# ricardo0115/p-div-gnn

Measured on AMD Instinct MI355X. Metric: mesh-nodes/sec (fwd+bwd) on periodic FEM graphs, higher is better.
Workload: dtype f32

## Files before the change

include/pdivgnn.h:

```cpp
#ifndef PDIVGNN_H
#define PDIVGNN_H

#include <stdint.h>

#ifdef __cplusplus
extern "C" {
#endif

#define PDG_LATENT 128
#define PDG_OK 0
#define PDG_ERR_ARG 1
#define PDG_ERR_HIP 2

typedef struct pdg_ln_stat {
  float mean;
  float den;
  float rstd;
  float std_;
  double mean_d, std_d, count;
} pdg_ln_stat;

typedef struct pdg_ln_bwd {
  float c1, c2;
  double S1, S2;
// ... 22 lines not shown
int pdg_ln_partials_sum(const double* partials, int nparts, double* out2, void* stream);

int pdg_node_pq(int n_nodes, const float* a2_prev, const pdg_ln_stat* st, const float* ln_g,
                const float* ln_b, const float* x_res, float* x_out, const float* W1,
                float* P, float* Q, void* stream);
int pdg_node_pq_rw(int n_nodes, const float* a2_prev, const pdg_ln_stat* st, const float* ln_g,
                   const float* ln_b, const float* x_res, float* x_out, const float* W1, float* P,
                   float* Q, void* stream);
int pdg_node_pq_rw_fin(int n_nodes, const float* a2_prev, const double* partials, int nparts, double count,
                       pdg_ln_stat* st_out, const float* ln_g, const float* ln_b, const float* x_res,
                       float* x_out, const float* W1, float* P, float* Q, void* stream);

int pdg_edge_fwd(int n_edges, const float* a2_prev, const pdg_ln_stat* st, const float* ln_g,
                 const float* ln_b, const float* e_res, float* e_out, const int* src, const int* dst,
                 const float* P, const float* Q, const float* W1, const float* b1,
                 const float* W2, const float* b2, float* a1m, float* a2m, float* a1e, float* a2e,
                 double* part_m, double* part_e, int with_edge_update, int* nparts, void* stream);

int pdg_segment_sum(int n_nodes, const int* rowptr, const float* rows, const pdg_ln_stat* st,
                    const float* ln_g, const float* ln_b, float* out, float* xhat_sum, void* stream);
int pdg_segment_sum_fin(int n_nodes, const int* rowptr, const float* rows, const double* part_a,
                        const double* part_b, int nparts, double count, pdg_ln_stat* st_a, pdg_ln_stat* st_b,
                        const float* ln_g, const float* ln_b, float* out, float* xhat_sum, void* stream);

int pdg_node_mlp1(int n_nodes, const float* aggr, const float* x, const float* Wn1,
                  const float* bn1, float* a1n, void* stream);

int pdg_mlp2_fwd(int rows, const float* a1, const float* W2, const float* b2, float* a2,
                 double* partials, int* nparts, void* stream);

int pdg_node_net(int n_nodes, const float* aggr, const float* x, const float* Wn1, const float* bn1,
                 const float* Wn2, const float* bn2, float* a1n, float* a2n, double* partials,
                 int* nparts, void* stream);
int pdg_decoder_fwd(int n_nodes, const float* a2_prev, const pdg_ln_stat* st, const float* ln_g,
                    const float* ln_b, const float* x_res, float* x_out, const float* Wd1,
                    const float* bd1, float* a1d, const float* Wd2, const float* bd2,
                    const float* stats8, int scale_output, float* y, void* stream);
int pdg_decoder_fwd_fin(int n_nodes, const float* a2_prev, const double* partials, int nparts, double count,
                        pdg_ln_stat* st_out, const float* ln_g, const float* ln_b, const float* x_res,
                        float* x_out, const float* Wd1, const float* bd1, float* a1d, const float* Wd2,
                        const float* bd2, const float* stats8, int scale_output, float* y, void* stream);
int pdg_decoder_fwd_coop(int n_nodes, const float* a2_prev, const pdg_ln_stat* st, const double* partials,
                         int nparts, double count, pdg_ln_stat* st_out, const float* ln_g, const float* ln_b,
                         const float* x_res, float* x_out, const float* Wd1, const float* bd1, float* a1d,
                         const float* Wd2, const float* bd2, const float* stats8, int scale_output, float* y,
                         int nblocks, void* stream);

int pdg_any_nonzero(const float* x, int64_t n, int* flag, void* stream);

int pdg_zero_unless(const int* flag, float* y, int64_t n, void* stream);


int pdg_decoder_bwd(int n_nodes, const float* gy, const float* a1d, const float* Wd2,
                    const float* Wd1T, float* gz1d, float* gx, void* stream);

int pdg_ln_colsum(int rows, const float* gy_rows, const int* gidx, const float* a2,
                  const pdg_ln_stat* st, double* partials, int* nparts, const float* ln_g,
                  double* pairs, int accumulate, void* stream);

int pdg_ln_colsum_nodes(int n_nodes, const float* gaggr, const int* rowptr, const float* xhat_sum,
                        double* partials, int* nparts, const float* ln_g, double* pairs, int accumulate,
                        void* stream);

int pdg_ln_colsum_finalize(const double* partials, int nparts, const float* ln_g,
                           const pdg_ln_stat* st, float* grad_g, float* grad_b, pdg_ln_bwd* out,
                           void* stream);
// ... 182 lines not shown
```

p-div-gnn_amd/csrc/pdg_common.hpp:

```cpp
#pragma once
#include <hip/hip_runtime.h>
#include <stdint.h>

#include "../../include/pdivgnn.h"
#include "pdg_runtime.hpp"

namespace pdg {

constexpr int L = 128;
constexpr int TILE = 16;
constexpr int FRAG = 32;
constexpr int WPAD = 136;
constexpr int WBLK = 128 * WPAD;
#ifndef PDG_EDGE_WAVES
#define PDG_EDGE_WAVES 12
#endif
constexpr int EDGE_WAVES = PDG_EDGE_WAVES;
constexpr float LN_EPS = 1e-5f;

typedef float f32x4 __attribute__((ext_vector_type(4)));
typedef unsigned u32x4 __attribute__((ext_vector_type(4)));

typedef pdg_ln_stat LNStat;
typedef pdg_ln_bwd LNBwd;
// ... 43 lines not shown
#endif
constexpr int PQ_LD = PDG_PQ_BLOCKED ? 2 * 128 : 128;
__device__ __forceinline__ int pq_col(int c) { return PDG_PQ_BLOCKED ? c + (c & ~15) : c; }

__device__ __forceinline__ __amdgpu_buffer_rsrc_t rows_rsrc(float* base, int r0, int r1) {
  return __builtin_amdgcn_make_buffer_rsrc(base ? base + (size_t)r0 * L : nullptr, (short)0,
                                           base ? (r1 - r0) * L * 4 : 0, 0x00020000);
}
__device__ __forceinline__ void rows_store4(__amdgpu_buffer_rsrc_t rs, int r, int c, const f32x4& v) {
  __builtin_amdgcn_raw_buffer_store_b128(__builtin_bit_cast(u32x4, v), rs, (r * L + c) * 4, 0, 0);
}
__device__ __forceinline__ void rows_store4_nt(__amdgpu_buffer_rsrc_t rs, int r, int c, const f32x4& v) {
  __builtin_amdgcn_raw_buffer_store_b128(__builtin_bit_cast(u32x4, v), rs, (r * L + c) * 4, 0, 2);
}

__device__ __forceinline__ void stnt4(float* __restrict__ p, const f32x4& x) { st4(p, 0, x); }
__device__ __forceinline__ float div_den(float x, float den, float rstd) {
  const float q = x * rstd;
  const float r = fmaf(-q, den, x);
  return fmaf(r, rstd, q);
}

template <bool RES>
__device__ __forceinline__ f32x4 ln_res4(const f32x4& x, const f32x4& r, const LNStat& st, const f32x4& g,
                                         const f32x4& b) {
  f32x4 y;
#pragma unroll
  for (int j = 0; j < 4; ++j) {
    float v = div_den(x[j] - st.mean, st.den, st.rstd) * g[j] + b[j];
    if (RES) v += r[j];
    y[j] = v;
  }
  return y;
}

__device__ __forceinline__ void load_wblock(float* __restrict__ lds, const float* __restrict__ W,
                                            int ld, int col0) {
  for (int idx = threadIdx.x; idx < 128 * 32; idx += blockDim.x) {
    const int o = idx >> 5, c4 = idx & 31;
    const f32x4 val = *reinterpret_cast<const f32x4*>(W + (size_t)o * ld + col0 + 4 * c4);
    *reinterpret_cast<f32x4*>(lds + o * WPAD + 4 * c4) = val;
  }
}

struct Acc {
  f32x4 b[8];
};
#define ACC(acc, s) (acc).b[(s) >> 2][(s) & 3]
#define PDG_FOR_FRAG(s) _Pragma("unroll") for (int s = 0; s < FRAG; ++s)
#define PDG_FENCE() __builtin_amdgcn_sched_barrier(0)

__device__ __forceinline__ void zero_acc(Acc& acc) {
#pragma unroll
  for (int ob = 0; ob < 8; ++ob) acc.b[ob] = f32x4{0.f, 0.f, 0.f, 0.f};
}

struct FeatVec {
  float lo, hi;
};
__device__ __forceinline__ FeatVec load_featvec(const float* __restrict__ p) {
  const int l = lane_id();
  return FeatVec{p[l], p[64 + l]};
}
__device__ __forceinline__ f32x4 featvec_chunk(const FeatVec& fv, int T) {
  const int addr = opaque(4 * (16 * (T & 3) + 4 * (lane_id() >> 4)));
  const int src = __float_as_int(T < 4 ? fv.lo : fv.hi);
// ... 295 lines not shown
```

p-div-gnn_amd/csrc/pdg_fwd.hip:

```cpp
#include <stdarg.h>
#include <stdio.h>

#include "pdg_common.hpp"
#include "pdg_runtime.hpp"

using namespace pdg;

namespace pdg {

static thread_local char g_err[512];

void set_error(const char* fmt, ...) {
  va_list ap;
  va_start(ap, fmt);
  vsnprintf(g_err, sizeof(g_err), fmt, ap);
  va_end(ap);
}

int device_cus() {
  static int cached[64] = {0};
  int dev = 0;
  (void)hipGetDevice(&dev);
  if (dev < 0 || dev >= 64) dev = 0;
  if (!cached[dev]) {
// ... 464 lines not shown
  __shared__ double red[8];
  if (part_a) {
    if (blockIdx.x == 0 && part_b) {
      ln_stat_from_partials(part_b, nparts, count, st_b, red);
      __syncthreads();
    }
    ln_stat_from_partials(part_a, nparts, count, &st_sh, red);
    __syncthreads();
    if (blockIdx.x == 0 && threadIdx.x == 0) *st_a = st_sh;
    stp = &st_sh;
  }
  const bool ln = stp != nullptr;
  if (ln) {
    mean = stp->mean;
    den = stp->den;
    rstd = stp->rstd;
    g = reinterpret_cast<const f32x4*>(lg)[j];
    b = reinterpret_cast<const f32x4*>(lb)[j];
  }
  for (int v = blockIdx.x * nhw + hw; v < N; v += gridDim.x * nhw) {
    const int k0 = rowptr[v], k1 = rowptr[v + 1];
    f32x4 acc = {0.f, 0.f, 0.f, 0.f}, xs = {0.f, 0.f, 0.f, 0.f};
    for (int k = k0; k < k1; k += SEG_U) {
      f32x4 x[SEG_U];
#pragma unroll
      for (int u = 0; u < SEG_U; ++u) {
        const int kk = k + u < k1 ? k + u : k1 - 1;
        x[u] = reinterpret_cast<const f32x4*>(rows + (size_t)kk * L)[j];
      }
#pragma unroll
      for (int u = 0; u < SEG_U; ++u) {
        if (k + u >= k1) break;
        if (ln) {
#pragma unroll
          for (int c = 0; c < 4; ++c) {
            const float h = div_den(x[u][c] - mean, den, rstd);
            xs[c] += h;
            x[u][c] = h * g[c] + b[c];
          }
        }
        acc += x[u];
      }
    }
    stg4(out + (size_t)v * L + 4 * j, acc);
    if (xsum) stg4(xsum + (size_t)v * L + 4 * j, xs);
  }
}

extern "C" int pdg_segment_sum(int n_nodes, const int* rowptr, const float* rows, const pdg_ln_stat* st,
                               const float* ln_g, const float* ln_b, float* out, float* xhat_sum, void* stream) {
  PDG_CHECK_ARG(!xhat_sum || (st && PDG_ALIGNED(xhat_sum)), "pdg_segment_sum: xhat_sum needs st, 16-B alignment");
  PDG_CHECK_ARG(n_nodes > 0, "pdg_segment_sum: n_nodes must be > 0");
  PDG_CHECK_ARG(PDG_ALIGNED(rows) && PDG_ALIGNED(out), "pdg_segment_sum: misaligned pointer");
  long want = (n_nodes + 7) / 8;
  long cap = (long)device_cus() * 8;
  const int grid = (int)(want < cap ? want : cap);
  hipLaunchKernelGGL(segment_sum_kernel, dim3(grid), dim3(256), 0, (hipStream_t)stream, n_nodes, rowptr, rows,
                     st, ln_g, ln_b, out, xhat_sum, nullptr, nullptr, 0, 0.0, nullptr, nullptr);
  PDG_CHECK_LAUNCH("pdg_segment_sum");
  return PDG_OK;
}

extern "C" int pdg_segment_sum_fin(int n_nodes, const int* rowptr, const float* rows, const double* part_a,
                                   const double* part_b, int nparts, double count, pdg_ln_stat* st_a,
                                   pdg_ln_stat* st_b, const float* ln_g, const float* ln_b, float* out,
                                   float* xhat_sum, void* stream) {
  PDG_CHECK_ARG(n_nodes > 0, "pdg_segment_sum_fin: n_nodes must be > 0");
  PDG_CHECK_ARG(part_a && st_a && ln_g && ln_b && nparts > 0 && nparts <= MAX_BLOCKS && count > 0 &&
                    (!part_b || st_b),
                "pdg_segment_sum_fin: bad statistics arguments");
  PDG_CHECK_ARG(PDG_ALIGNED(rows) && PDG_ALIGNED(out) && (!xhat_sum || PDG_ALIGNED(xhat_sum)),
                "pdg_segment_sum_fin: misaligned pointer");
// ... 231 lines not shown
```

p-div-gnn_amd/csrc/pdg_node.hip:

```cpp
#include "pdg_common.hpp"
#include "pdg_runtime.hpp"
#include "pdg_x6.hpp"

using namespace pdg;

namespace {

constexpr int NU_COMPUTE = 8;
constexpr int NU_LOADERS = 4;
constexpr int NU_THREADS = 64 * (NU_COMPUTE + NU_LOADERS);
constexpr int XS = 2 * L + 8;
constexpr int AS = L + 8;
constexpr int XBUF = TILE * XS;

struct TileRegs {
  f32x4 v[4];
};

__device__ __forceinline__ void fetch_tile(TileRegs& tr, int t, int N, int lt, const float* __restrict__ aggr,
                                           const float* __restrict__ x) {
  const int j = lt & 31, lr = lt >> 5;
#pragma unroll
  for (int u = 0; u < 4; ++u) {
    const int r = lr + 8 * (u >> 1), node = t * TILE + r;
// ... 105 lines not shown
    }
    stage((i + 2) % 3);
  }
  __shared__ double red[2 * NU_COMPUTE];
  block_sum2(s1, s2, red);
  if (threadIdx.x == 0) {
    part[2 * blockIdx.x] = s1;
    part[2 * blockIdx.x + 1] = s2;
  }
}



extern "C" int pdg_node_net(int n_nodes, const float* aggr, const float* x, const float* Wn1, const float* bn1,
                            const float* Wn2, const float* bn2, float* a1n, float* a2n, double* partials,
                            int* nparts, void* stream) {
  PDG_CHECK_ARG(n_nodes > 0, "pdg_node_net: n_nodes must be > 0");
  PDG_CHECK_ARG(n_nodes < (1 << 22), "pdg_node_net: at most 4,194,303 nodes per call");
  PDG_CHECK_ARG(aggr && x && a2n, "pdg_node_net: aggr, x and a2n are required");
  PDG_CHECK_ARG(PDG_ALIGNED(aggr) && PDG_ALIGNED(x) && PDG_ALIGNED(Wn1) && PDG_ALIGNED(Wn2) && PDG_ALIGNED(a2n) &&
                    PDG_ALIGNED(a1n) && PDG_ALIGNED(bn1) && PDG_ALIGNED(bn2),
                "pdg_node_net: misaligned pointer");
  const int tiles = tiles_of(n_nodes);
  const int cap = device_cus() < MAX_BLOCKS ? device_cus() : MAX_BLOCKS;
  const int grid = tiles < cap ? tiles : cap;
  hipLaunchKernelGGL(node_net_x6_kernel, dim3(grid), dim3(64 * NU_COMPUTE), 0, (hipStream_t)stream, n_nodes, aggr, x,
                     Wn1, bn1, Wn2, bn2, a1n, a2n, partials);
  PDG_CHECK_LAUNCH("pdg_node_net");
  if (nparts) *nparts = grid;
  return PDG_OK;
}

namespace {

constexpr int GS = L + 8;

struct Gz2Regs {
  f32x4 gv[2], av[2];
};

__device__ __forceinline__ void fetch_gz2(Gz2Regs& rg, int t, int N, int lt, const float* __restrict__ gy,
                                          const float* __restrict__ a2) {
#pragma unroll
  for (int u = 0; u < 2; ++u) {
    const int c = lt + 256 * u, rr = c >> 5, j = c & 31, node = t * TILE + rr;
    const bool ok = node < N;
    rg.gv[u] = ok ? reinterpret_cast<const f32x4*>(gy + (size_t)node * L)[j] : f32x4{0.f, 0.f, 0.f, 0.f};
    rg.av[u] = ok ? reinterpret_cast<const f32x4*>(a2 + (size_t)node * L)[j] : f32x4{0.f, 0.f, 0.f, 0.f};
  }
}

__device__ __forceinline__ void store_gz2(float* __restrict__ buf, float* __restrict__ gybuf, int t, int N, int lt,
                                          const Gz2Regs& rg, const LNStat& st, const pdg_ln_bwd& lb,
                                          const float* __restrict__ g, float* __restrict__ gz2_out) {
#pragma unroll
  for (int u = 0; u < 2; ++u) {
    const int c = lt + 256 * u, rr = c >> 5, j = c & 31, node = t * TILE + rr;
    const f32x4 gg = reinterpret_cast<const f32x4*>(g)[j];
    f32x4 z;
#pragma unroll
    for (int e = 0; e < 4; ++e) {
      const float xhat = div_den(rg.av[u][e] - st.mean, st.den, st.rstd);
      const float ga = st.rstd * (gg[e] * rg.gv[u][e] - lb.c1) - xhat * lb.c2;
      z[e] = rg.av[u][e] > 0.f ? ga : 0.f;
    }
    *reinterpret_cast<f32x4*>(buf + rr * GS + 4 * j) = z;
// ... 370 lines not shown
```

p-div-gnn_amd/pdg/engine.py:

```python
from __future__ import annotations

import ctypes
import os
from dataclasses import dataclass, field

import torch

from . import hiptimer
from .lib import LN_STAT_BYTES, lib, stream_handle
from .lib import ptr as _p
from .plan import GraphPlan

L = 128
VP, IA = ctypes.c_void_p, ctypes.c_int


def _arr(ctype, values):
    values = list(values)
    return (ctype * len(values))(*values)


PARAM_SHAPES = [
    ("node_encoder.0.weight", (L, 6)), ("node_encoder.0.bias", (L,)),
    ("node_encoder.2.weight", (L, L)), ("node_encoder.2.bias", (L,)),
    ("node_encoder.4.weight", (L,)), ("node_encoder.4.bias", (L,)),
    ("edge_encoder.0.weight", (L, 1)), ("edge_encoder.0.bias", (L,)),
    ("edge_encoder.2.weight", (L, L)), ("edge_encoder.2.bias", (L,)),
    ("edge_encoder.4.weight", (L,)), ("edge_encoder.4.bias", (L,)),
    ("processor.edge_net.0.weight", (L, 3 * L)), ("processor.edge_net.0.bias", (L,)),
    ("processor.edge_net.2.weight", (L, L)), ("processor.edge_net.2.bias", (L,)),
    ("processor.edge_net.4.weight", (L,)), ("processor.edge_net.4.bias", (L,)),
    ("processor.node_net.0.weight", (L, 2 * L)), ("processor.node_net.0.bias", (L,)),
    ("processor.node_net.2.weight", (L, L)), ("processor.node_net.2.bias", (L,)),
    ("processor.node_net.4.weight", (L,)), ("processor.node_net.4.bias", (L,)),
    ("node_decoder.0.weight", (L, L)), ("node_decoder.0.bias", (L,)),
    ("node_decoder.2.weight", (3, L)), ("node_decoder.2.bias", (3,)),
]
PARAM_NAMES = [n for n, _ in PARAM_SHAPES]


VARIANTS = {
    "fused_edge_wgrad": ("PDG_FUSED_EDGE_WGRAD", True),
    "gz1e_from_gc": ("PDG_GZ1E_FROM_GC", True),
    "coop_fwd": ("PDG_EDGE_FWD_COOP", True),
    "pair_blocks_per_cu": ("PDG_PAIR_BLOCKS_PER_CU", 1),
    "enc_blocks_per_cu": ("PDG_ENC_BLOCKS_PER_CU", 2),
}


INFER_PIPE_MIN_EDGES = 32768


def _parse_variant(name: str, raw: str):
    env, default = VARIANTS[name]
    if isinstance(default, bool):
        if raw not in ("0", "1"):
            raise ValueError(f"{env}={raw!r}: expected 0 or 1")
        return raw == "1"
    try:
        v = int(raw)
    except ValueError:
        raise ValueError(f"{env}={raw!r}: expected an integer") from None
    if v < 1 or v > 4:
        raise ValueError(f"{env}={raw!r}: expected 1..4")
    return v


def kernel_variants(overrides: dict | None = None) -> dict:
    out = {k: d for k, (_, d) in VARIANTS.items()}
    ab = os.environ.get("PDG_AB") == "1"
    for name, (env, default) in VARIANTS.items():
        raw = os.environ.get(env)
        if raw is None:
            continue
        val = _parse_variant(name, raw)
        if val != default and not ab:
            raise RuntimeError(f"{env}={raw} selects a non-default kernel variant of the HIP path; these are "
# ... 90 lines not shown
    n_node: int = 0
    sync_slot: int = 0

    def PN(self, t):
        return self.pairs[t]

    def PM(self, t):
        return self.pairs[self.S + t]

    def PE(self, t):
        return self.pairs[2 * self.S + t]


_DEFERRED = [
    ("W2", "processor.edge_net.2.weight", L, 0, "processor.edge_net.2.bias"),
    ("Wc", "processor.edge_net.0.weight", 3 * L, 2 * L, "processor.edge_net.0.bias"),
    ("Wn2", "processor.node_net.2.weight", L, 0, "processor.node_net.2.bias"),
    ("d1", "node_decoder.0.weight", L, 0, "node_decoder.0.bias"),
    ("ne2", "node_encoder.2.weight", L, 0, "node_encoder.2.bias"),
    ("ee2", "edge_encoder.2.weight", L, 0, "edge_encoder.2.bias"),
]


class EPDEngine:

    def __init__(self, device: torch.device, variants: dict | None = None) -> None:
        self.device = torch.device(device)
        var = kernel_variants(variants)
        self.max_blocks = lib.pdg_max_blocks()
        self._cus = torch.cuda.get_device_properties(self.device).multi_processor_count
        f64 = dict(dtype=torch.float64, device=self.device)
        self._part_a = torch.empty(self.max_blocks * 2, **f64)
        self._part_b = torch.empty(self.max_blocks * 2, **f64)
        self._part_col = torch.empty(self.max_blocks * 256, **f64)
        self._acc_rows = min(2 * self._cus, self.max_blocks)
        self._ln_acc = torch.zeros(4, self._acc_rows * 256, **f64)
        self._sync_pairs = torch.zeros(8, 2, **f64)
        self._part_narrow = torch.empty(self.max_blocks * (L * 6 + L + 6), **f64)
        self._part_narrow_d = torch.empty(self.max_blocks * (L * 3 + L + 3), **f64)
        self._part_narrow_ne = torch.empty(self.max_blocks * (L * 6 + L + 6), **f64)
        self._nparts = ctypes.c_int(0)
        self._nslabs = lib.pdg_wgrad_slabs_per_cu() * self._cus
        self._nslabs_p = min(var["pair_blocks_per_cu"] * self._cus, self.max_blocks)
        self._nslabs_e = min(self._cus, self.max_blocks)
        self._enc_blocks = min(var["enc_blocks_per_cu"] * self._cus, self.max_blocks)
        self._pair = torch.zeros(2, **f64)
        self._slab_sets: dict = {}
        self._slabs_p = None
        self.sync = None
        for k, v in var.items():
            if isinstance(v, bool):
                setattr(self, k, v)
        self.pq_blocked = bool(lib.pdg_pq_layout())
        self.timed: dict | None = None
        self.probe: dict | None = None

    def variants(self) -> dict:
        derived = {"pair_blocks_per_cu": self._nslabs_p // self._cus,
                   "enc_blocks_per_cu": self._enc_blocks // self._cus}
        return {k: derived[k] if k in derived else getattr(self, k) for k in VARIANTS}

    def _t(self, name: str, fn, *args):
        if self.timed is None or name not in self.timed:
            return fn(*args)
        a, b = hiptimer.Event(), hiptimer.Event()
        a.record()
# ... 78 lines not shown

    def _fwd_step(self, P, f: _Fwd, t: int) -> None:
        ctx, s, st, need_grad = f.ctx, f.s, f.ctx.stats, f.need_grad
        plan = ctx.plan
        N, E = plan.n_nodes, plan.n_edges
        i_m, i_e, i_n = 2 + 3 * t, 3 + 3 * t, 4 + 3 * t
        ge, be = P["processor.edge_net.4.weight"], P["processor.edge_net.4.bias"]
        gn, bnn = P["processor.node_net.4.weight"], P["processor.node_net.4.bias"]
        a2n_prev, stn_prev, gn_prev, bn_prev = f.ln_n
        x_t = self._empty(N, L)
        if f.pend_n is not None:
            self._t("node_pq", lib.pdg_node_pq_rw_fin, N, _p(a2n_prev), f.pend_buf.data_ptr(), f.pend_n,
                    float(N * L), stn_prev, _p(gn_prev), _p(bn_prev), _p(f.x), _p(x_t),
                    _p(P["processor.edge_net.0.weight"]), _p(f.Pm), _p(f.Qm), s)
            f.pend_n = None
        else:
            self._t("node_pq", lib.pdg_node_pq_rw, N, _p(a2n_prev), stn_prev, _p(gn_prev), _p(bn_prev),
                    _p(f.x), _p(x_t), _p(P["processor.edge_net.0.weight"]), _p(f.Pm), _p(f.Qm), s)
        eu = t < ctx.steps - 1
        e_t = self._empty(E, L)
        a2m = self._empty(E, L)
        a1m = self._empty(E, L) if need_grad else None
        a2e = self._empty(E, L) if eu else None
        a1e = self._empty(E, L) if (eu and need_grad) else None
        fin_in_segsum = bool(E) and self.sync is None
        if E:
            self._fwd_edge_net(P, f, eu, e_t, a1m, a2m, a1e, a2e)
        if E and not fin_in_segsum:
            self._finalize(self._part_a, E * L, st[i_m], s, True)
            if eu:
                self._finalize(self._part_b, E * L, st[i_e], s, True)
        a1n = self._empty(N, L) if need_grad else None
        a2n = self._empty(N, L)
        if E:
            aggr = self._empty(N, L)
            xs = self._empty(N, L) if need_grad else None
            if fin_in_segsum:
                self._t("segment_sum", lib.pdg_segment_sum_fin, N, _p(plan.rowptr_dst), _p(a2m),
                        _p(self._part_a), _p(self._part_b) if eu else None, self._nparts.value, float(E * L),
                        st[i_m], st[i_e] if eu else None, _p(ge), _p(be), _p(aggr), _p(xs), s)
            else:
                self._t("segment_sum", lib.pdg_segment_sum, N, _p(plan.rowptr_dst), _p(a2m), st[i_m], _p(ge),
                        _p(be), _p(aggr), _p(xs), s)
        else:
            aggr = torch.zeros(N, L, dtype=torch.float32, device=self.device)
            xs = torch.zeros(N, L, dtype=torch.float32, device=self.device) if need_grad else None
        self._t("node_net", lib.pdg_node_net, N, _p(aggr), _p(x_t), _p(P["processor.node_net.0.weight"]),
                _p(P["processor.node_net.0.bias"]), _p(P["processor.node_net.2.weight"]),
                _p(P["processor.node_net.2.bias"]), _p(a1n), _p(a2n), _p(self._part_a),
                ctypes.byref(self._nparts), s)
        if self.sync is None:
            f.pend_n, f.pend_buf = self._nparts.value, self._part_a
        else:
            self._finalize(self._part_a, N * L, st[i_n], s)
        if need_grad:
            ctx.per_step.append(dict(x=x_t, e=e_t, a1m=a1m, a2m=a2m, a1e=a1e, a2e=a2e, aggr=aggr, xs=xs,
                                     a1n=a1n, a2n=a2n, i_m=i_m, i_e=i_e, i_n=i_n, eu=eu))
        f.ln_n = (a2n, st[i_n], gn, bnn)
        f.ln_e = (a2e, st[i_e], ge, be)
        f.x, f.e = x_t, e_t

    def _fwd_edge_net(self, P, f: _Fwd, eu: bool, e_t, a1m, a2m, a1e, a2e) -> None:
        plan, s = f.ctx.plan, f.s
        N, E = plan.n_nodes, plan.n_edges
        a2e_prev, ste_prev, ge_prev, be_prev = f.ln_e
        W1, b1 = P["processor.edge_net.0.weight"], P["processor.edge_net.0.bias"]
        W2, b2 = P["processor.edge_net.2.weight"], P["processor.edge_net.2.bias"]
        name = "edge_fwd" if eu else "edge_fwd_last"
        if self.coop_fwd and not f.need_grad and E >= INFER_PIPE_MIN_EDGES:
            self._t(name, lib.pdg_edge_fwd_infer, E, _p(a2e_prev), ste_prev, _p(ge_prev), _p(be_prev), _p(f.e),
                    _p(e_t), _p(plan.src), _p(plan.dst), _p(f.Pm), _p(f.Qm), _p(W1), _p(b1), _p(W2), _p(b2),
                    _p(a2m), _p(a2e), _p(self._part_a), _p(self._part_b), int(eu), self._nslabs_e, s)
            self._nparts.value = self._nslabs_e
        elif self.coop_fwd:
            self._t(name, lib.pdg_edge_fwd_coop, E, _p(a2e_prev), ste_prev, _p(ge_prev), _p(be_prev), _p(f.e),
                    _p(e_t), _p(plan.src), _p(plan.dst), _p(f.Pm), _p(f.Qm), _p(W1), _p(b1), _p(W2), _p(b2),
                    _p(a1m), _p(a2m), _p(a1e), _p(a2e), _p(self._part_a), _p(self._part_b), int(eu),
                    self._nslabs_e, s)
            self._nparts.value = self._nslabs_e
        else:
            Pu, Qu = f.Pm, f.Qm
            if self.pq_blocked:
                v = f.PQm.view(N, 8, 2, 16)
                Pu, Qu = v[:, :, 0].reshape(N, L).contiguous(), v[:, :, 1].reshape(N, L).contiguous()
            self._t(name, lib.pdg_edge_fwd, E, _p(a2e_prev), ste_prev, _p(ge_prev), _p(be_prev), _p(f.e),
                    _p(e_t), _p(plan.src), _p(plan.dst), _p(Pu), _p(Qu), _p(W1), _p(b1), _p(W2), _p(b2),
                    _p(a1m), _p(a2m), _p(a1e), _p(a2e), _p(self._part_a), _p(self._part_b), int(eu),
# ... 315 lines not shown
```

p-div-gnn_amd/pdg/lib.py:

```python
from __future__ import annotations

import ctypes
import hashlib
import os
from ctypes import c_double, c_float, c_int, c_int64, c_void_p
from pathlib import Path

import torch

SHIPPED = Path(__file__).resolve().parent / "libpdivgnn_hip.so"
LIB_PATH = Path(os.environ.get("PDG_LIB", SHIPPED))
CSRC = Path(__file__).resolve().parents[1] / "csrc"


def source_hash(csrc: Path = CSRC) -> str | None:
    files = sorted(csrc.glob("*.hip")) + sorted(csrc.glob("*.hpp")) + [csrc.parent.parent / "include" / "pdivgnn.h"]
    if not csrc.is_dir() or not files[-1].exists():
        return None
    h = hashlib.sha256()
    for f in files:
        h.update(f.name.encode())
        h.update(f.read_bytes())
    return h.hexdigest()[:16]

P = c_void_p
I = c_int

SIGNATURES: dict[str, list] = {
    "pdg_last_error": [],
    "pdg_version": [],
    "pdg_source_hash": [],
    "pdg_max_blocks": [],
    "pdg_pq_layout": [],
    "pdg_format_inputs": [I, I, P, P, P, P, P, P, I, P, P, P],
    "pdg_encoder_fwd": [I, I, P, P, P, P, P, P, P, P, P, P],
    "pdg_ln_finalize": [P, I, c_double, P, P],
    "pdg_ln_finalize2": [P, P, I, c_double, P, P, P],
    "pdg_node_pq_rw_fin": [I, P, P, I, c_double, P, P, P, P, P, P, P, P, P],
    "pdg_ln_partials_sum": [P, I, P, P],
    "pdg_node_pq": [I, P, P, P, P, P, P, P, P, P, P],
    "pdg_node_pq_rw": [I, P, P, P, P, P, P, P, P, P, P],
    "pdg_edge_fwd": [I, P, P, P, P, P, P, P, P, P, P, P, P, P, P, P, P, P, P, P, P, I, P, P],
    "pdg_segment_sum": [I, P, P, P, P, P, P, P, P],
    "pdg_segment_sum_fin": [I, P, P, P, P, I, c_double, P, P, P, P, P, P, P],
    "pdg_node_mlp1": [I, P, P, P, P, P, P],
    "pdg_mlp2_fwd": [I, P, P, P, P, P, P, P],
    "pdg_node_net": [I, P, P, P, P, P, P, P, P, P, P, P],
    "pdg_decoder_fwd": [I, P, P, P, P, P, P, P, P, P, P, P, P, I, P, P],
    "pdg_decoder_fwd_fin": [I, P, P, I, c_double, P] + [P] * 10 + [I, P, P],
    "pdg_decoder_fwd_coop": [I, P, P, P, I, c_double, P] + [P] * 10 + [I, P, I, P],
    "pdg_any_nonzero": [P, c_int64, P, P],
    "pdg_zero_unless": [P, P, c_int64, P],
    "pdg_decoder_bwd": [I, P, P, P, P, P, P, P],
    "pdg_ln_colsum": [I, P, P, P, P, P, P, P, P, I, P],
    "pdg_ln_colsum_nodes": [I, P, P, P, P, P, P, P, I, P],
    "pdg_ln_colsum_finalize": [P, I, P, P, P, P, P, P],
    "pdg_ln_param_grads": [I, P, P, P, P, P],
    "pdg_mlp2_bwd": [I, P, P, P, P, P, P, P, P, P, P, P, I, P],
    "pdg_node_bwd": [I, P, P, P, P, P, P, P, P, P, P, P, P, P, P, I, P],
    "pdg_gemm_dual": [I, P, P, P, P, P, P, P, P],
    "pdg_gemm_sum2": [I, P, P, P, P, P, P, P],
    "pdg_gemm_sum2_rw": [I, P, P, P, P, P, P, P, P, P, P, P, P, I, P],
    "pdg_edge_bwd": [I, P, P, P, P, P, P, P, P, P, P, P, P, P, P, P, P, P, P, P, P, P, I, P, I, P],
    "pdg_pq_scatter_bwd": [I, P, P, P, P, P, I, P, P, P],
    "pdg_wgrad_accum": [I, P, P, P, P, P, I, P],
    "pdg_wgrad_reduce": [P, I, P, I, I, P, P],
    "pdg_transpose128_batch": [I, P, P, P, P],
    "pdg_wgrad_reduce_batch": [I, P, P, P, P, P, P, P],
    "pdg_wgrad_segments_batch": [I, P, P, P, P, P, I, P],
    "pdg_edge_fwd_coop": [I, P, P, P, P, P, P, P, P, P, P, P, P, P, P, P, P, P, P, P, P, I, I, P],
    "pdg_edge_fwd_infer": [I, P, P, P, P, P, P, P, P, P, P, P, P, P, P, P, P, P, P, I, I, P],
    "pdg_edge_enc_fwd": [I, P, P, P, P, P, P, P, I, P],
    "pdg_node_enc_fwd": [I, P, P, P, P, P, P, P, P, I, P],
    "pdg_gemm_sum2_coop": [I, P, P, P, P, P, P, P, P, P, P, P, I, I, P],
    "pdg_node_bwd_coop": [I] + [P] * 14 + [I, I, P],
    "pdg_mlp2_bwd_coop": [I] + [P] * 10 + [I, P, P, I, P],
    "pdg_decoder_bwd_coop": [I] + [P] * 11 + [I, P, I, P],
    "pdg_wgrad_narrow_finalize": [P, I, I, I, P, P, P, P],
    "pdg_bwd_epilogue": [I, P, P, P, P, P, P, I, P, P, P, P, I, P, P, P, P, P, P, P, P, I, P, P, P],
    "pdg_wgrad_slabs_per_cu": [],
# ... 106 lines not shown
```

Measured before the change: 5.153 million.

## Fuse LayerNorm segment-sum aggregation into the node MLP kernel

```diff
diff --git a/include/pdivgnn.h b/include/pdivgnn.h
--- a/include/pdivgnn.h
+++ b/include/pdivgnn.h
@@ -78,6 +78,15 @@
 int pdg_node_net(int n_nodes, const float* aggr, const float* x, const float* Wn1, const float* bn1,
                  const float* Wn2, const float* bn2, float* a1n, float* a2n, double* partials,
                  int* nparts, void* stream);
+int pdg_node_net_agg(int n_nodes, int n_edges, const int* rowptr, const float* rows, const pdg_ln_stat* st,
+                     const float* ln_g, const float* ln_b, float* aggr, float* xhat_sum, const float* x,
+                     const float* Wn1, const float* bn1, const float* Wn2, const float* bn2, float* a1n,
+                     float* a2n, double* partials, int* nparts, void* stream);
+int pdg_node_net_agg_fin(int n_nodes, int n_edges, const int* rowptr, const float* rows, const double* part_a,
+                         const double* part_b, int nparts_in, double count, pdg_ln_stat* st_a,
+                         pdg_ln_stat* st_b, const float* ln_g, const float* ln_b, float* aggr, float* xhat_sum,
+                         const float* x, const float* Wn1, const float* bn1, const float* Wn2, const float* bn2,
+                         float* a1n, float* a2n, double* partials, int* nparts, void* stream);
 int pdg_decoder_fwd(int n_nodes, const float* a2_prev, const pdg_ln_stat* st, const float* ln_g,
                     const float* ln_b, const float* x_res, float* x_out, const float* Wd1,
                     const float* bd1, float* a1d, const float* Wd2, const float* bd2,
diff --git a/p-div-gnn_amd/csrc/pdg_common.hpp b/p-div-gnn_amd/csrc/pdg_common.hpp
--- a/p-div-gnn_amd/csrc/pdg_common.hpp
+++ b/p-div-gnn_amd/csrc/pdg_common.hpp
@@ -99,6 +99,15 @@
     y[j] = v;
   }
   return y;
+}
+
+__device__ __forceinline__ void seg_row_terms(const f32x4& x, float mean, float den, float rstd, const f32x4& g,
+                                              const f32x4& b, f32x4& h, f32x4& y) {
+#pragma unroll
+  for (int c = 0; c < 4; ++c) {
+    h[c] = div_den(x[c] - mean, den, rstd);
+    y[c] = h[c] * g[c] + b[c];
+  }
 }
 
 __device__ __forceinline__ void load_wblock(float* __restrict__ lds, const float* __restrict__ W,
diff --git a/p-div-gnn_amd/csrc/pdg_fwd.hip b/p-div-gnn_amd/csrc/pdg_fwd.hip
--- a/p-div-gnn_amd/csrc/pdg_fwd.hip
+++ b/p-div-gnn_amd/csrc/pdg_fwd.hip
@@ -520,12 +520,9 @@
       for (int u = 0; u < SEG_U; ++u) {
         if (k + u >= k1) break;
         if (ln) {
-#pragma unroll
-          for (int c = 0; c < 4; ++c) {
-            const float h = div_den(x[u][c] - mean, den, rstd);
-            xs[c] += h;
-            x[u][c] = h * g[c] + b[c];
-          }
+          f32x4 h;
+          seg_row_terms(x[u], mean, den, rstd, g, b, h, x[u]);
+          xs += h;
         }
         acc += x[u];
       }
diff --git a/p-div-gnn_amd/csrc/pdg_node.hip b/p-div-gnn_amd/csrc/pdg_node.hip
--- a/p-div-gnn_amd/csrc/pdg_node.hip
+++ b/p-div-gnn_amd/csrc/pdg_node.hip
@@ -161,6 +161,222 @@
 }
 
 namespace {
+__device__ __forceinline__ float uniform(float x) {
+  return __int_as_float(__builtin_amdgcn_readfirstlane(__float_as_int(x)));
+}
+}
+
+#ifndef PDG_NA_U
+#define PDG_NA_U 4
+#endif
+constexpr int NA_U = PDG_NA_U;
+
+__global__ __launch_bounds__(64 * NU_COMPUTE, 1) void node_net_agg_x6_kernel(
+    int N, int E, const int* __restrict__ rowptr, const float* __restrict__ rows,
+    const pdg_ln_stat* __restrict__ stp, const float* __restrict__ lg, const float* __restrict__ lb,
+    float* __restrict__ aggr_out, float* __restrict__ xs_out, const float* __restrict__ x,
+    const float* __restrict__ W1, const float* __restrict__ b1, const float* __restrict__ W2,
+    const float* __restrict__ b2, float* __restrict__ a1_out, float* __restrict__ a2_out,
+    double* __restrict__ part, const double* __restrict__ part_a, const double* __restrict__ part_b, int nparts_in,
+    double count, pdg_ln_stat* __restrict__ st_a, pdg_ln_stat* __restrict__ st_b) {
+  __shared__ __attribute__((aligned(16))) unsigned char xin[3 * 2 * NN_IMG];
+  __shared__ __attribute__((aligned(16))) unsigned char a1i[2 * NN_IMG];
+  __shared__ pdg_ln_stat st_sh;
+  __shared__ double red[2 * NU_COMPUTE];
+  __shared__ f32x4 lnp[64];
+  const int w = wave_id(), l = lane_id();
+  const int ntiles = tiles_of(N);
+  if (part_a) {
+    if (blockIdx.x == 0 && part_b) {
+      ln_stat_from_partials(part_b, nparts_in, count, st_b, red);
+      __syncthreads();
+    }
+    ln_stat_from_partials(part_a, nparts_in, count, &st_sh, red);
+    __syncthreads();
+    if (blockIdx.x == 0 && threadIdx.x == 0) *st_a = st_sh;
+    stp = &st_sh;
+  }
+  const int r = l & 15, q = l >> 4;
+  const int oc = 16 * w + 4 * q;
+  const int j = threadIdx.x & 31, rr = threadIdx.x >> 5;
+  const float mean = uniform(stp->mean), den = uniform(stp->den), rstd = uniform(stp->rstd);
+  if (threadIdx.x < 64)
+    lnp[threadIdx.x] = reinterpret_cast<const f32x4*>(threadIdx.x < 32 ? lg : lb)[threadIdx.x & 31];
+  __syncthreads();
+  const __amdgpu_buffer_rsrc_t rs_a1 = rows_rsrc(a1_out, 0, N), rs_a2 = rows_rsrc(a2_out, 0, N);
+  const __amdgpu_buffer_rsrc_t rs_ag = rows_rsrc(aggr_out, 0, N), rs_xs = rows_rsrc(xs_out, 0, N);
+  int k0 = 0, k1 = 0, nk0, nk1, srow;
+  f32x4 xr[NA_U], vx;
+  bool vok;
+  auto seg_rows = [&](int k) {
+#pragma unroll
+    for (int u = 0; u < NA_U; ++u) {
+      const int kk = min(max(k + u < k1 ? k + u : k1 - 1, 0), E - 1);
+      xr[u] = reinterpret_cast<const f32x4*>(rows + (size_t)kk * L)[j];
+    }
+  };
+  auto bounds = [&](int t, int& a, int& b) {
+    const int node = clamp_row(t * TILE + rr, N);
+    a = rowptr[node];
+    b = rowptr[node + 1];
+  };
+  auto fetch = [&](int t) {
+    const int node = t * TILE + rr;
+    vok = node < N;
+    srow = vok ? node : N;
+    seg_rows(k0);
+    vx = reinterpret_cast<const f32x4*>(x + (size_t)clamp_row(node, N) * L)[j];
+  };
+  f32x4 acc, xs;
+  const f32x4 zero = f32x4{0.f, 0.f, 0.f, 0.f};
+  auto add_rows = [&](int k) {
+#pragma unroll
+    for (int u = 0; u < NA_U; ++u) pin_vgpr(xr[u]);
+    const int jj = opaque(j);
+    const f32x4 gg = lnp[jj], bb = lnp[32 + jj];
+#pragma unroll
+    for (int u = 0; u < NA_U; ++u) {
+      f32x4 h, y;
+      seg_row_terms(xr[u], mean, den, rstd, gg, bb, h, y);
+      const bool on = k + u < k1;
+#pragma unroll
+      for (int c = 0; c < 4; ++c) {
+        xs[c] += on ? h[c] : 0.f;
+        acc[c] += on ? y[c] : 0.f;
+      }
+    }
+  };
+  auto mid = [&](int buf) {
+    acc = zero;
+    xs = zero;
+    add_rows(k0);
+    seg_rows(k0 + NA_U);
+    x6_store4<NN_T16>(xin + (2 * buf + 1) * NN_IMG, rr, j, vok ? vx : zero);
+  };
+  auto stage = [&](int buf) {
+    add_rows(k0 + NA_U);
+    for (int k = k0 + 2 * NA_U; k < k1; k += NA_U) {
+      seg_rows(k);
+      add_rows(k);
+    }
+    rows_store4(rs_ag, srow, 4 * j, acc);
+    rows_store4(rs_xs, srow, 4 * j, xs);
+    x6_store4<NN_T16>(xin + (2 * buf) * NN_IMG, rr, j, vok ? acc : zero);
+  };
+  bounds(nu_tile(0), k0, k1);
+  bounds(nu_tile(1), nk0, nk1);
+  fetch(nu_tile(0));
+  mid(0);
+  stage(0);
+  k0 = nk0;
+  k1 = nk1;
+  bounds(nu_tile(2), nk0, nk1);
+  if (nu_tile(1) < ntiles) {
+    fetch(nu_tile(1));
+    mid(1);
+    stage(1);
+  }
+  k0 = nk0;
+  k1 = nk1;
+  WSlice w1a, w1b, w2;
+  load_wslice(w1a, W1, w, 2 * L);
+  load_wslice(w1b, W1 + L, w, 2 * L);
+  load_wslice(w2, W2, w, L);
+  const f32x4 bias1 = *reinterpret_cast<const f32x4*>(b1 + oc);
+  const f32x4 bias2 = *reinterpret_cast<const f32x4*>(b2 + oc);
+  double s1 = 0, s2 = 0;
+  __syncthreads();
+  for (int i = 0;; ++i) {
+    const int tile = nu_tile(i);
+    if (tile >= ntiles) break;
+    fetch(nu_tile(i + 2));
+    bounds(nu_tile(i + 3), nk0, nk1);
+    const int row = tile * TILE + r;
+    f32x4 d1[1] = {{0.f, 0.f, 0.f, 0.f}};
+    gemm_x6f<1, NN_T16, true>(d1, w1a, xin + (2 * (i % 3)) * NN_IMG);
+    gemm_x6f<1, NN_T16, true>(d1, w1b, xin + (2 * (i % 3) + 1) * NN_IMG);
+    f32x4 a1;
+#pragma unroll
+    for (int c = 0; c < 4; ++c) a1[c] = fmaxf(d1[0][c] + bias1[c], 0.f);
+    x6_store4<NN_T16>(a1i + (i & 1) * NN_IMG, r, 4 * w + q, a1);
+    rows_store4(rs_a1, row, oc, a1);
+    __syncthreads();
+    mid((i + 2) % 3);
+    f32x4 d2[1] = {{0.f, 0.f, 0.f, 0.f}};
+    gemm_x6f<1, NN_T16, true>(d2, w2, a1i + (i & 1) * NN_IMG);
+    f32x4 a2;
+#pragma unroll
+    for (int c = 0; c < 4; ++c) a2[c] = fmaxf(d2[0][c] + bias2[c], 0.f);
+    rows_store4(rs_a2, row, oc, a2);
+    if (row < N) {
+      const float p1 = (a2[0] + a2[1]) + (a2[2] + a2[3]);
+      const float p2 = (a2[0] * a2[0] + a2[1] * a2[1]) + (a2[2] * a2[2] + a2[3] * a2[3]);
+      s1 += (double)p1;
+      s2 += (double)p2;
+    }
+    stage((i + 2) % 3);
+    k0 = nk0;
+    k1 = nk1;
+  }
+  block_sum2(s1, s2, red);
+  if (threadIdx.x == 0) {
+    part[2 * blockIdx.x] = s1;
+    part[2 * blockIdx.x + 1] = s2;
+  }
+}
+
+static int node_net_agg_launch(const char* who, int n_nodes, int n_edges, const int* rowptr, const float* rows,
+                               const pdg_ln_stat* st, const float* ln_g, const float* ln_b, float* aggr,
+                               float* xhat_sum, const float* x, const float* Wn1, const float* bn1,
+                               const float* Wn2, const float* bn2, float* a1n, float* a2n, double* partials,
+                               int* nparts, const double* part_a, const double* part_b, int nparts_in,
+                               double count, pdg_ln_stat* st_a, pdg_ln_stat* st_b, void* stream) {
+  PDG_CHECK_ARG(n_nodes > 0 && n_edges > 0, "pdg_node_net_agg: n_nodes and n_edges must be > 0");
+  PDG_CHECK_ARG(n_nodes < (1 << 22), "pdg_node_net_agg: at most 4,194,303 nodes per call");
+  PDG_CHECK_ARG(rowptr && rows && ln_g && ln_b && x && Wn1 && bn1 && Wn2 && bn2 && a2n && partials,
+                "pdg_node_net_agg: null argument");
+  PDG_CHECK_ARG(PDG_ALIGNED(rows) && PDG_ALIGNED(ln_g) && PDG_ALIGNED(ln_b) && PDG_ALIGNED(aggr) &&
+                    PDG_ALIGNED(xhat_sum) && PDG_ALIGNED(x) && PDG_ALIGNED(Wn1) && PDG_ALIGNED(bn1) &&
+                    PDG_ALIGNED(Wn2) && PDG_ALIGNED(bn2) && PDG_ALIGNED(a1n) && PDG_ALIGNED(a2n),
+                "pdg_node_net_agg: misaligned pointer");
+  const int tiles = tiles_of(n_nodes);
+  const int cap = device_cus() < MAX_BLOCKS ? device_cus() : MAX_BLOCKS;
+  const int grid = tiles < cap ? tiles : cap;
+  hipLaunchKernelGGL(node_net_agg_x6_kernel, dim3(grid), dim3(64 * NU_COMPUTE), 0, (hipStream_t)stream, n_nodes,
+                     n_edges, rowptr, rows, st, ln_g, ln_b, aggr, xhat_sum, x, Wn1, bn1, Wn2, bn2, a1n, a2n, partials,
+                     part_a, part_b, nparts_in, count, st_a, st_b);
+  PDG_CHECK_LAUNCH(who);
+  if (nparts) *nparts = grid;
+  return PDG_OK;
+}
+
+extern "C" int pdg_node_net_agg(int n_nodes, int n_edges, const int* rowptr, const float* rows,
+                                const pdg_ln_stat* st, const float* ln_g, const float* ln_b, float* aggr,
+                                float* xhat_sum, const float* x, const float* Wn1, const float* bn1,
+                                const float* Wn2, const float* bn2, float* a1n, float* a2n, double* partials,
+                                int* nparts, void* stream) {
+  PDG_CHECK_ARG(st != nullptr, "pdg_node_net_agg: null argument (st)");
+  return node_net_agg_launch("pdg_node_net_agg", n_nodes, n_edges, rowptr, rows, st, ln_g, ln_b, aggr, xhat_sum, x,
+                             Wn1, bn1, Wn2, bn2, a1n, a2n, partials, nparts, nullptr, nullptr, 0, 0.0, nullptr,
+                             nullptr, stream);
+}
+
+extern "C" int pdg_node_net_agg_fin(int n_nodes, int n_edges, const int* rowptr, const float* rows,
+                                    const double* part_a, const double* part_b, int nparts_in, double count,
+                                    pdg_ln_stat* st_a, pdg_ln_stat* st_b, const float* ln_g, const float* ln_b,
+                                    float* aggr, float* xhat_sum, const float* x, const float* Wn1,
+                                    const float* bn1, const float* Wn2, const float* bn2, float* a1n, float* a2n,
+                                    double* partials, int* nparts, void* stream) {
+  PDG_CHECK_ARG(part_a && st_a && nparts_in > 0 && nparts_in <= MAX_BLOCKS && count > 0 && (!part_b || st_b),
+                "pdg_node_net_agg_fin: bad statistics arguments");
+  PDG_CHECK_ARG(partials != part_a && partials != part_b,
+                "pdg_node_net_agg_fin: partials must not alias part_a / part_b");
+  return node_net_agg_launch("pdg_node_net_agg_fin", n_nodes, n_edges, rowptr, rows, nullptr, ln_g, ln_b, aggr,
+                             xhat_sum, x, Wn1, bn1, Wn2, bn2, a1n, a2n, partials, nparts, part_a, part_b, nparts_in,
+                             count, st_a, st_b, stream);
+}
+
+namespace {
 
 constexpr int GS = L + 8;
 
diff --git a/p-div-gnn_amd/pdg/engine.py b/p-div-gnn_amd/pdg/engine.py
--- a/p-div-gnn_amd/pdg/engine.py
+++ b/p-div-gnn_amd/pdg/engine.py
@@ -43,6 +43,7 @@
     "fused_edge_wgrad": ("PDG_FUSED_EDGE_WGRAD", True),
     "gz1e_from_gc": ("PDG_GZ1E_FROM_GC", True),
     "coop_fwd": ("PDG_EDGE_FWD_COOP", True),
+    "node_net_agg": ("PDG_NODE_NET_AGG", True),
     "pair_blocks_per_cu": ("PDG_PAIR_BLOCKS_PER_CU", 1),
     "enc_blocks_per_cu": ("PDG_ENC_BLOCKS_PER_CU", 2),
 }
@@ -199,6 +200,7 @@
         f64 = dict(dtype=torch.float64, device=self.device)
         self._part_a = torch.empty(self.max_blocks * 2, **f64)
         self._part_b = torch.empty(self.max_blocks * 2, **f64)
+        self._part_n = torch.empty(self.max_blocks * 2, **f64)
         self._part_col = torch.empty(self.max_blocks * 256, **f64)
         self._acc_rows = min(2 * self._cus, self.max_blocks)
         self._ln_acc = torch.zeros(4, self._acc_rows * 256, **f64)
@@ -343,27 +345,42 @@
                 self._finalize(self._part_b, E * L, st[i_e], s, True)
         a1n = self._empty(N, L) if need_grad else None
         a2n = self._empty(N, L)
-        if E:
-            aggr = self._empty(N, L)
+        part_n = self._part_a
+        Wn1, bn1 = P["processor.node_net.0.weight"], P["processor.node_net.0.bias"]
+        Wn2, bn2 = P["processor.node_net.2.weight"], P["processor.node_net.2.bias"]
+        if E and self.node_net_agg:
+            aggr = self._empty(N, L) if need_grad else None
             xs = self._empty(N, L) if need_grad else None
             if fin_in_segsum:
-                self._t("segment_sum", lib.pdg_segment_sum_fin, N, _p(plan.rowptr_dst), _p(a2m),
-                        _p(self._part_a), _p(self._part_b) if eu else None, self._nparts.value, float(E * L),
-                        st[i_m], st[i_e] if eu else None, _p(ge), _p(be), _p(aggr), _p(xs), s)
+                part_n = self._part_n
+                self._t("node_net", lib.pdg_node_net_agg_fin, N, E, _p(plan.rowptr_dst), _p(a2m), _p(self._part_a),
+                        _p(self._part_b) if eu else None, self._nparts.value, float(E * L), st[i_m],
+                        st[i_e] if eu else None, _p(ge), _p(be), _p(aggr), _p(xs), _p(x_t), _p(Wn1), _p(bn1),
+                        _p(Wn2), _p(bn2), _p(a1n), _p(a2n), _p(part_n), ctypes.byref(self._nparts), s)
             else:
-                self._t("segment_sum", lib.pdg_segment_sum, N, _p(plan.rowptr_dst), _p(a2m), st[i_m], _p(ge),
-                        _p(be), _p(aggr), _p(xs), s)
-        else:
-            aggr = torch.zeros(N, L, dtype=torch.float32, device=self.device)
-            xs = torch.zeros(N, L, dtype=torch.float32, device=self.device) if need_grad else None
-        self._t("node_net", lib.pdg_node_net, N, _p(aggr), _p(x_t), _p(P["processor.node_net.0.weight"]),
-                _p(P["processor.node_net.0.bias"]), _p(P["processor.node_net.2.weight"]),
-                _p(P["processor.node_net.2.bias"]), _p(a1n), _p(a2n), _p(self._part_a),
-                ctypes.byref(self._nparts), s)
+                self._t("node_net", lib.pdg_node_net_agg, N, E, _p(plan.rowptr_dst), _p(a2m), st[i_m], _p(ge),
+                        _p(be), _p(aggr), _p(xs), _p(x_t), _p(Wn1), _p(bn1), _p(Wn2), _p(bn2), _p(a1n), _p(a2n),
+                        _p(part_n), ctypes.byref(self._nparts), s)
+        else:
+            if E:
+                aggr = self._empty(N, L)
+                xs = self._empty(N, L) if need_grad else None
+                if fin_in_segsum:
+                    self._t("segment_sum", lib.pdg_segment_sum_fin, N, _p(plan.rowptr_dst), _p(a2m),
+                            _p(self._part_a), _p(self._part_b) if eu else None, self._nparts.value, float(E * L),
+                            st[i_m], st[i_e] if eu else None, _p(ge), _p(be), _p(aggr), _p(xs), s)
+                else:
+                    self._t("segment_sum", lib.pdg_segment_sum, N, _p(plan.rowptr_dst), _p(a2m), st[i_m], _p(ge),
+                            _p(be), _p(aggr), _p(xs), s)
+            else:
+                aggr = torch.zeros(N, L, dtype=torch.float32, device=self.device)
+                xs = torch.zeros(N, L, dtype=torch.float32, device=self.device) if need_grad else None
+            self._t("node_net", lib.pdg_node_net, N, _p(aggr), _p(x_t), _p(Wn1), _p(bn1), _p(Wn2), _p(bn2), _p(a1n),
+                    _p(a2n), _p(part_n), ctypes.byref(self._nparts), s)
         if self.sync is None:
-            f.pend_n, f.pend_buf = self._nparts.value, self._part_a
-        else:
-            self._finalize(self._part_a, N * L, st[i_n], s)
+            f.pend_n, f.pend_buf = self._nparts.value, part_n
+        else:
+            self._finalize(part_n, N * L, st[i_n], s)
         if need_grad:
             ctx.per_step.append(dict(x=x_t, e=e_t, a1m=a1m, a2m=a2m, a1e=a1e, a2e=a2e, aggr=aggr, xs=xs,
                                      a1n=a1n, a2n=a2n, i_m=i_m, i_e=i_e, i_n=i_n, eu=eu))
diff --git a/p-div-gnn_amd/pdg/lib.py b/p-div-gnn_amd/pdg/lib.py
--- a/p-div-gnn_amd/pdg/lib.py
+++ b/p-div-gnn_amd/pdg/lib.py
@@ -46,6 +46,8 @@
     "pdg_node_mlp1": [I, P, P, P, P, P, P],
     "pdg_mlp2_fwd": [I, P, P, P, P, P, P, P],
     "pdg_node_net": [I, P, P, P, P, P, P, P, P, P, P, P],
+    "pdg_node_net_agg": [I, I] + [P] * 17,
+    "pdg_node_net_agg_fin": [I, I, P, P, P, P, I, c_double] + [P] * 16,
     "pdg_decoder_fwd": [I, P, P, P, P, P, P, P, P, P, P, P, P, I, P, P],
     "pdg_decoder_fwd_fin": [I, P, P, I, c_double, P] + [P] * 10 + [I, P, P],
     "pdg_decoder_fwd_coop": [I, P, P, P, I, c_double, P] + [P] * 10 + [I, P, I, P],
```

New measurement: 5.187 million (median of 6 runs). About the same (+0.7%).
